# krukah/robopoker

Hardware: AMD Instinct MI355X
Metric: mccfr_infoset_updates_per_sec (higher is better)
Workload: dtype f32; 1 GPU; leduc-holdem external-sampling MCCFR, tables resident in HBM (BASELINE configs[1]); regret=floored, weight=linear, sampling=external, batch_per_gpu=8388608, global_batch=8388608, infosets=120, actions=2, update=composed, parallelism=tree-sharded x1

## Files before the change

include/rp_mi355x.h:

```cpp
#ifndef RP_MI355X_H
#define RP_MI355X_H

#include <stddef.h>
#include <stdint.h>

#ifdef __cplusplus
extern "C" {
#endif

#define RP_API __attribute__((visibility("default")))

typedef enum rp_status {
    RP_OK = 0,
    RP_ERR_INVALID = 1,
    RP_ERR_NO_DEVICE = 2,
    RP_ERR_HIP = 3,
    RP_ERR_UNSUPPORTED = 4,
    RP_ERR_CAPACITY = 5,
    RP_ERR_INTERNAL = 6
} rp_status;

RP_API const char* rp_last_error(void);
RP_API int rp_device_count(void);
RP_API const char* rp_version(void);
// ... 125 lines not shown
RP_API int rp_mccfr_get(rp_mccfr* h, uint32_t info, uint32_t edge, rp_encounter* out);
RP_API int rp_mccfr_set(rp_mccfr* h, uint32_t info, uint32_t edge, const rp_encounter* in);
RP_API int rp_mccfr_export(rp_mccfr* h, rp_encounter* rows, uint64_t cap);
RP_API int rp_mccfr_import(rp_mccfr* h, const rp_encounter* rows, uint64_t n, uint64_t epoch);
typedef enum rp_dist_kind {
    RP_DIST_ITERATED = 0,
    RP_DIST_AVERAGED = 1,
    RP_DIST_SAMPLING = 2
} rp_dist_kind;
RP_API int rp_mccfr_policy(rp_mccfr* h, uint32_t info, rp_dist_kind kind, float* out, uint32_t* n);
RP_API int rp_mccfr_exploitability(rp_mccfr* h, float* out);
RP_API int rp_mccfr_sum_regret(rp_mccfr* h, float* out);
RP_API int rp_mccfr_set_batch(rp_mccfr* h, uint32_t batch_size);
RP_API int rp_mccfr_set_update_mode(rp_mccfr* h, rp_update_mode mode);
RP_API int rp_mccfr_set_stream(rp_mccfr* h, void* hip_stream);

RP_API int rp_mccfr_set_shard(rp_mccfr* h, uint32_t rank, uint32_t world);
RP_API int rp_mccfr_summary_bytes(rp_mccfr* h, size_t* bytes);
RP_API int rp_mccfr_step_local(rp_mccfr* h, void* summary_dev);
RP_API int rp_mccfr_step_apply(rp_mccfr* h, const void* gathered_dev, uint32_t world);
RP_API int rp_mccfr_window_local(rp_mccfr* h, void* window_dev, int first);
RP_API int rp_mccfr_window_apply(rp_mccfr* h, const void* gathered_dev, uint32_t world);

#define RP_COMM_ID_BYTES 128
typedef struct rp_comm rp_comm;
RP_API int rp_comm_unique_id(uint8_t* id );
RP_API int rp_comm_create(const uint8_t* id, int rank, int world, int device, rp_comm** out);
RP_API int rp_comm_adopt(void* nccl_comm, int rank, int world, int device, rp_comm** out);
RP_API int rp_comm_destroy(rp_comm* c);
RP_API int rp_mccfr_step_comm(rp_mccfr* h, rp_comm* c, uint32_t steps, uint32_t window);

RP_API int rp_mccfr_traversal_variant(rp_mccfr* h, int* out);
RP_API int rp_mccfr_traversal_rows_bytes(rp_mccfr* h, size_t* out);
RP_API int rp_game_skeleton(const rp_game_table* game, int* out);

#define RP_SPARSE_BLOCK 64u
typedef struct rp_profile rp_profile;
typedef struct rp_decisions {
    uint32_t n;
    const uint32_t* row;
    const uint8_t* n_actions;
    const uint16_t* expanded;
    const float* regret;
    const float* policy;
    const float* payoff;
} rp_decisions;
RP_API int rp_profile_create(int device, uint64_t n_rows, uint32_t max_actions, rp_regret_kind regret,
                             rp_weight_kind weight, const rp_hyper* hp, const float* default_regret,
                             uint32_t max_batch, rp_profile** out);
RP_API int rp_profile_destroy(rp_profile* h);
RP_API int rp_profile_apply(rp_profile* h, const rp_decisions* batch, rp_update_mode mode);
RP_API int rp_profile_sync(rp_profile* h);
RP_API int rp_profile_epoch(const rp_profile* h, uint64_t* epoch);
RP_API int rp_profile_set_epoch(rp_profile* h, uint64_t epoch);
RP_API int rp_profile_get_rows(rp_profile* h, uint64_t n, const uint32_t* rows, rp_encounter* out);
RP_API int rp_profile_set_rows(rp_profile* h, uint64_t n, const uint32_t* rows, const rp_encounter* in);
RP_API int rp_profile_policy(rp_profile* h, rp_dist_kind kind, uint64_t n, const uint32_t* rows_dev, const uint8_t* n_actions_dev,
                             float* policy_dev);
RP_API int rp_profile_set_stream(rp_profile* h, void* hip_stream);
RP_API int rp_profile_entry_bytes(const rp_profile* h, size_t* bytes);
RP_API int rp_profile_summarize(rp_profile* h, const rp_decisions* batch, void* entries_dev, uint32_t* n_entries);
RP_API int rp_profile_fold(rp_profile* h, const void* entries_dev, uint32_t n_entries);

typedef struct rp_nlhe rp_nlhe;
typedef struct rp_lookup rp_lookup;
RP_API int rp_nlhe_create(int device, uint32_t cap_log2, rp_regret_kind regret, rp_weight_kind weight, const rp_hyper* hp,
// ... 465 lines not shown
```

robopoker_amd/_lib.py:

```python
from __future__ import annotations

import ctypes as C
import os

_HERE = os.path.dirname(os.path.abspath(__file__))
LIB_PATH = os.path.join(_HERE, "librp_mi355x.so")

RP_OK = 0
RP_ERR_INVALID = 1
RP_ERR_NO_DEVICE = 2
RP_ERR_HIP = 3
RP_ERR_UNSUPPORTED = 4
RP_ERR_CAPACITY = 5

RP_TURN_CHANCE = 254
RP_TURN_TERMINAL = 255
RP_NO_INFO = 0xFFFFFFFF

REGRET = {"summed": 0, "linear": 1, "discounted": 2, "floored": 3, "asymmetric": 4}
WEIGHT = {"constant": 0, "linear": 1, "quadratic": 2, "exponential": 3}
SAMPLING = {"external": 0, "prunable": 1, "pluribus": 2}
GAME = {"kuhn": 0, "leduc": 1, "rps": 2, "leduc_wide": 3}
DIST = {"iterated": 0, "averaged": 1, "sampling": 2}
METRIC = {"sinkhorn": 0, "variation": 1}
# ... 248 lines not shown
    "rp_game_table_check": (C.c_int, [C.POINTER(GameTable)]),
    "rp_mccfr_create": (
        C.c_int,
        [C.POINTER(GameTable), C.c_int, C.c_int, C.c_int, C.c_uint32, C.POINTER(Hyper), C.c_uint64, C.c_int,
         C.POINTER(C.c_void_p)],
    ),
    "rp_mccfr_create_mode": (
        C.c_int,
        [C.POINTER(GameTable), C.c_int, C.c_int, C.c_int, C.c_uint32, C.POINTER(Hyper), C.c_uint64, C.c_int, C.c_int,
         C.POINTER(C.c_void_p)],
    ),
    "rp_mccfr_destroy": (C.c_int, [C.c_void_p]),
    "rp_mccfr_step": (C.c_int, [C.c_void_p]),
    "rp_mccfr_solve": (C.c_int, [C.c_void_p, C.c_uint64]),
    "rp_mccfr_spend": (C.c_int, [C.c_void_p, C.c_double, C.POINTER(C.c_uint64), C.POINTER(C.c_double)]),
    "rp_mccfr_step_async": (C.c_int, [C.c_void_p, C.c_uint32]),
    "rp_mccfr_sync": (C.c_int, [C.c_void_p]),
    "rp_mccfr_epoch": (C.c_int, [C.c_void_p, C.POINTER(C.c_uint64)]),
    "rp_mccfr_counters": (C.c_int, [C.c_void_p, C.POINTER(C.c_uint64), C.POINTER(C.c_uint64)]),
    "rp_mccfr_get": (C.c_int, [C.c_void_p, C.c_uint32, C.c_uint32, C.POINTER(Encounter)]),
    "rp_mccfr_set": (C.c_int, [C.c_void_p, C.c_uint32, C.c_uint32, C.POINTER(Encounter)]),
    "rp_mccfr_export": (C.c_int, [C.c_void_p, C.POINTER(Encounter), C.c_uint64]),
    "rp_mccfr_import": (C.c_int, [C.c_void_p, C.POINTER(Encounter), C.c_uint64, C.c_uint64]),
    "rp_mccfr_policy": (C.c_int, [C.c_void_p, C.c_uint32, C.c_int, C.POINTER(C.c_float), C.POINTER(C.c_uint32)]),
    "rp_mccfr_exploitability": (C.c_int, [C.c_void_p, C.POINTER(C.c_float)]),
    "rp_mccfr_sum_regret": (C.c_int, [C.c_void_p, C.POINTER(C.c_float)]),
    "rp_mccfr_set_batch": (C.c_int, [C.c_void_p, C.c_uint32]),
    "rp_mccfr_set_update_mode": (C.c_int, [C.c_void_p, C.c_int]),
    "rp_mccfr_set_rng": (C.c_int, [C.c_void_p, C.c_int, C.POINTER(HashStreams)]),
    "rp_game_hash_streams": (C.c_int, [C.c_void_p, C.POINTER(HashStreams)]),
    "rp_mccfr_set_stream": (C.c_int, [C.c_void_p, C.c_void_p]),
    "rp_mccfr_traversal_variant": (C.c_int, [C.c_void_p, C.POINTER(C.c_int)]),
    "rp_mccfr_traversal_rows_bytes": (C.c_int, [C.c_void_p, C.POINTER(C.c_size_t)]),
    "rp_game_skeleton": (C.c_int, [C.c_void_p, C.POINTER(C.c_int)]),
    "rp_mccfr_set_shard": (C.c_int, [C.c_void_p, C.c_uint32, C.c_uint32]),
    "rp_mccfr_summary_bytes": (C.c_int, [C.c_void_p, C.POINTER(C.c_size_t)]),
    "rp_mccfr_step_local": (C.c_int, [C.c_void_p, C.c_void_p]),
    "rp_mccfr_step_apply": (C.c_int, [C.c_void_p, C.c_void_p, C.c_uint32]),
    "rp_mccfr_window_local": (C.c_int, [C.c_void_p, C.c_void_p, C.c_int]),
    "rp_mccfr_window_apply": (C.c_int, [C.c_void_p, C.c_void_p, C.c_uint32]),
    "rp_comm_unique_id": (C.c_int, [C.c_void_p]),
    "rp_comm_create": (C.c_int, [C.c_void_p, C.c_int, C.c_int, C.c_int, C.POINTER(C.c_void_p)]),
    "rp_comm_adopt": (C.c_int, [C.c_void_p, C.c_int, C.c_int, C.c_int, C.POINTER(C.c_void_p)]),
    "rp_comm_destroy": (C.c_int, [C.c_void_p]),
    "rp_mccfr_step_comm": (C.c_int, [C.c_void_p, C.c_void_p, C.c_uint32, C.c_uint32]),
    "rp_kmeans_step_comm": (C.c_int, [C.c_void_p, C.c_void_p, C.c_void_p, C.c_void_p, C.POINTER(C.c_double)]),
    "rp_mccfr_profile": (C.c_int, [C.c_void_p, C.c_int]),
    "rp_mccfr_kernel_time": (C.c_int, [C.c_void_p, C.c_char_p, C.POINTER(C.c_double), C.POINTER(C.c_uint64)]),
    "rp_profile_create": (C.c_int, [C.c_int, C.c_uint64, C.c_uint32, C.c_int, C.c_int, C.POINTER(Hyper), C.c_void_p, C.c_uint32,
                                    C.POINTER(C.c_void_p)]),
    "rp_profile_destroy": (C.c_int, [C.c_void_p]),
    "rp_profile_apply": (C.c_int, [C.c_void_p, C.POINTER(Decisions), C.c_int]),
    "rp_profile_sync": (C.c_int, [C.c_void_p]),
    "rp_profile_epoch": (C.c_int, [C.c_void_p, C.POINTER(C.c_uint64)]),
    "rp_profile_set_epoch": (C.c_int, [C.c_void_p, C.c_uint64]),
    "rp_profile_get_rows": (C.c_int, [C.c_void_p, C.c_uint64, C.c_void_p, C.c_void_p]),
    "rp_profile_policy": (C.c_int, [C.c_void_p, C.c_int, C.c_uint64, C.c_void_p, C.c_void_p, C.c_void_p]),
    "rp_profile_set_stream": (C.c_int, [C.c_void_p, C.c_void_p]),
    "rp_profile_entry_bytes": (C.c_int, [C.c_void_p, C.POINTER(C.c_size_t)]),
    "rp_profile_summarize": (C.c_int, [C.c_void_p, C.POINTER(Decisions), C.c_void_p, C.POINTER(C.c_uint32)]),
    "rp_profile_fold": (C.c_int, [C.c_void_p, C.c_void_p, C.c_uint32]),
    "rp_profile_profile": (C.c_int, [C.c_void_p, C.c_int]),
    "rp_profile_kernel_time": (C.c_int, [C.c_void_p, C.c_char_p, C.POINTER(C.c_double), C.POINTER(C.c_uint64)]),
    "rp_sinkhorn_hp_default": (None, [C.POINTER(SinkhornHP)]),
    "rp_kmeans_create": (
        C.c_int,
# ... 183 lines not shown
```

robopoker_amd/csrc/mccfr.hip:

```cpp
#include "mccfr_kernels.hpp"
#include "mccfr_traverse.hpp"
#include "mccfr_update.hpp"
#include "traverse_static.hpp"

#include <algorithm>
#include <chrono>
#include <cstdlib>
#include <functional>
#include <string>
#include <type_traits>
#include <vector>

#define HIP_TRY(expr)                                                                                 \
    do {                                                                                              \
        hipError_t _e = (expr);                                                                       \
        if (_e != hipSuccess) return rp::fail(RP_ERR_HIP, "%s failed: %s", #expr, hipGetErrorString(_e)); \
    } while (0)

using namespace rp;

struct KernelClock {
    std::vector<std::pair<hipEvent_t, hipEvent_t>> pending;
    double total_ms = 0.0;
    uint64_t launches = 0;
// ... 22 lines not shown
    void* d_info_actions = nullptr;
    void* d_info_player = nullptr;
    void* d_info_rank = nullptr;
    void* d_scratch = nullptr;
    void* d_dec = nullptr;
    void* d_summary = nullptr;
    void* d_window = nullptr;
    uint32_t window_world = 0;
    void* d_sorted = nullptr;
    void* d_bmaps = nullptr;
    uint32_t maxint = 1;
    void* d_itab = nullptr;
    DevInfoTab itab{};
    DevSorted so{};
    unsigned long long* d_counters = nullptr;
    int R = 0, W = 0, S = 0;
    rp_hyper hp{};
    uint64_t seed = 0;
    rp_rng_kind rng = RP_RNG_COUNTER;
    uint32_t n_chance_infos = 0;
    void* d_info_streams = nullptr;
    void* d_chance_streams = nullptr;
    void* d_ref_mid = nullptr;
    uint64_t ref_mid_epoch = ~0ull;
    uint32_t batch = 1, capacity = 0;
    uint64_t epoch = 0;
    uint32_t rank = 0, world = 1;
    uint32_t maxdec = 1;
    rp_update_mode mode = RP_UPDATE_ORDERED;
    bool use_lds_traverse = false;
    uint64_t tables_version = 1, itab_version = 0;
    static constexpr uint32_t cell_pad = 7;
    bool fuse_maps = true;
    int static_skel = 0;
    bool profiling = false;
    KernelClock clk_traverse, clk_compact, clk_update;
};

namespace {

int set_device(const rp_mccfr* h) {
    HIP_TRY(hipSetDevice(h->device));
    return RP_OK;
}

size_t chain_lds_bytes() { return (size_t)CHAIN_LDS_WORDS * 4; }

size_t summary_bytes_of(const rp_mccfr* h) {
    return (size_t)h->tbl.n_infos * h->tbl.max_actions * sizeof(Cell) + (size_t)h->tbl.n_infos * sizeof(InfoSum);
}

void sampled_tree_bounds(const rp_mccfr* h, uint32_t* maxdec, uint32_t* maxstack, uint32_t* maxint) {
    const rp::TableBounds b = rp::table_bounds(h->tbl, h->tbl.train_root);
    *maxdec = std::max(b.decisions, 1u);
    *maxstack = std::max(b.stack, 1u) + 1;
    *maxint = std::max(b.internal, 1u);
}

size_t chunk_maps_lds_bytes(const rp_mccfr* h);
int alloc_batch_buffers(rp_mccfr* h, uint32_t batch) {
    if (batch <= h->capacity) return RP_OK;
    if (h->d_scratch) HIP_TRY(hipFree(h->d_scratch));
    if (h->d_dec) HIP_TRY(hipFree(h->d_dec));
    h->d_scratch = h->d_dec = nullptr;
    const size_t stride = ((size_t)batch + 255) & ~(size_t)255;
    const uint32_t A = h->tbl.max_actions;
// ... 294 lines not shown

int launch_chain(rp_mccfr* h, const StepParams& p) {
    const size_t lds = chain_lds_bytes();
    const bool sgn = h->R == RP_REGRET_DISCOUNTED || h->R == RP_REGRET_ASYMMETRIC;
    const bool prn = h->S != RP_SAMPLING_EXTERNAL;
    const dim3 grid(h->tbl.n_infos), block(128);
    clock_begin(h, h->clk_update);
    with_bools(sgn, prn, [&](auto sg, auto pr) {
        hipLaunchKernelGGL((k_chain<decltype(sg)::value, decltype(pr)::value>), grid, block, lds, h->stream, h->g, h->t, h->so, p);
    });
    clock_end(h, h->clk_update);
    HIP_TRY(hipGetLastError());
    return RP_OK;
}

uint32_t chunks_of(size_t trees) { return (uint32_t)((trees + RP_COMPOSE_CHUNK - 1) / RP_COMPOSE_CHUNK); }
size_t chunk_maps_lds_bytes(const rp_mccfr* h) {
    const size_t NI = h->tbl.n_infos;
    return NI * SM_WORDS * 4 + 2 * NI * 4 + (size_t)CH_TREES * h->maxdec * 4 + NI * SM_WORDS * 2 +
           2 * (size_t)CH_TREES * h->maxdec * 2;
}

size_t traverse_maps_lds_bytes(const rp_mccfr* h) {
    const size_t NI = h->tbl.n_infos;
    const size_t masks = h->S != RP_SAMPLING_EXTERNAL ? (size_t)h->maxdec * 256 * 4 : 0;
    return (NI * 8 + 2 * NI) * 4 + NI * 8 * 2 + (NI + (NI & 1)) * 2 + 2 * NI * 4 + (size_t)3 * (h->maxdec * 256 + h->cell_pad) * 4 + masks;
}
static_assert(CH_THREADS <= 256u, "k_traverse_maps_static packs (infoset, rank of the infoset) into the 16 bits of an `order` entry");
bool traverse_maps_fused(const rp_mccfr* h) {
    return h->static_skel && !h->dc.slotmap && h->tbl.n_infos <= CH_THREADS && h->g.rank_max <= 64u &&
           traverse_maps_lds_bytes(h) <= 64 * 1024 && h->fuse_maps;
}

int launch_summarize(rp_mccfr* h, const StepParams& p, void* blob_dev, bool fused = false, bool apply = false) {
    unsigned char* blob = reinterpret_cast<unsigned char*>(blob_dev);
    Cell* cells = reinterpret_cast<Cell*>(blob);
    InfoSum* sums = reinterpret_cast<InfoSum*>(blob + (size_t)h->tbl.n_infos * h->tbl.max_actions * sizeof(Cell));
    const uint32_t A = h->tbl.max_actions;
    const uint32_t nblk_max = chunks_of(h->dc.stride), nblk = chunks_of(h->batch);
    Map* bmaps = reinterpret_cast<Map*>(h->d_bmaps);
    const bool pruned = h->S != RP_SAMPLING_EXTERNAL;
    if (fused) {
        clock_begin(h, h->clk_traverse);
        launch_prepare(h, p);
        const size_t lds = traverse_maps_lds_bytes(h);
        with_static_traversal(h->static_skel, p.walker, pruned, p.ref_info != nullptr, [&](auto gt, auto wk, auto pr, auto rf) {
            hipLaunchKernelGGL((k_traverse_maps_static<decltype(gt), decltype(wk)::value, decltype(pr)::value, decltype(rf)::value>), dim3(nblk),
                               dim3(256), lds, h->stream, h->g, h->itab, p, bmaps, h->maxdec, h->cell_pad);
        });
        clock_end(h, h->clk_traverse);
    }
    clock_begin(h, h->clk_update);
    if (fused) {
    } else if (!h->dc.slotmap) {
        const size_t lds = chunk_maps_lds_bytes(h);
        with_bools(pruned, h->tbl.n_infos <= CH_THREADS, [&](auto pr, auto one) {
            hipLaunchKernelGGL((k_chunk_maps<decltype(pr)::value, decltype(one)::value ? 1u : CM_PASSES>), dim3(nblk), dim3(CH_THREADS), lds,
                               h->stream, h->g, h->dc, p, bmaps);
        });
    } else {
        with_bool(pruned, [&](auto pr) {
            hipLaunchKernelGGL((k_block_maps<decltype(pr)::value>), dim3(nblk, h->tbl.n_infos), dim3(128), 0, h->stream, h->g, h->so, p, bmaps);
        });
    }
    {
        const uint32_t W2 = 2 * A, nr = h->g.rank_count[p.walker];
        const uint32_t ngrp_max = (nblk_max + RP_FOLD_GROUP - 1) / RP_FOLD_GROUP, ngrp = (nblk + RP_FOLD_GROUP - 1) / RP_FOLD_GROUP;
        FoldScratch fs;
        fs.gmaps = bmaps + bmap_index(nblk_max, 0, 0, h->g.rank_max, W2);
        fs.done = reinterpret_cast<uint32_t*>(bmaps + bmap_index(nblk_max + ngrp_max, 0, 0, h->g.rank_max, W2));
        const dim3 grid(std::max(ngrp, 1u), cb2_tiles(nr, W2));
        if (apply) {
            hipLaunchKernelGGL((k_combine2<true>), grid, dim3(CB2_THREADS), 0, h->stream, h->g, h->t, h->itab, p, bmaps, nr, fs, cells, sums);
            h->tables_version += 1;
            if (h->itab_version + 1 == h->tables_version) h->itab_version = h->tables_version;
        } else {
            hipLaunchKernelGGL((k_combine2<false>), grid, dim3(CB2_THREADS), 0, h->stream, h->g, h->t, h->itab, p, bmaps, nr, fs, cells, sums);
        }
    }
    clock_end(h, h->clk_update);
    HIP_TRY(hipGetLastError());
    return RP_OK;
}

int launch_batch_summary(rp_mccfr* h, const StepParams& p, void* blob_dev, bool apply = false) {
    if (traverse_maps_fused(h)) return launch_summarize(h, p, blob_dev, true, apply);
    int rc = launch_traverse(h, p);
    if (rc) return rc;
    if (h->dc.slotmap && (rc = launch_sort(h, p))) return rc;
    return launch_summarize(h, p, blob_dev, false, apply);
}

int enqueue_step(rp_mccfr* h) {
    const StepParams p = make_params(h);
    int rc;
    if (h->mode == RP_UPDATE_ORDERED) {
        if ((rc = launch_traverse(h, p))) return rc;
        if ((rc = launch_sort(h, p))) return rc;
        if ((rc = launch_chain(h, p))) return rc;
        h->tables_version += 1;
    } else {
        if ((rc = launch_batch_summary(h, p, h->d_summary, true))) return rc;
    }
    h->epoch += 1;
    return RP_OK;
}

int read_counters(rp_mccfr* h, unsigned long long c[3]) {
    std::vector<unsigned long long> all((size_t)METRIC_STRIPES * METRIC_STRIDE);
    HIP_TRY(hipMemcpyAsync(all.data(), h->d_counters, all.size() * 8, hipMemcpyDeviceToHost, h->stream));
// ... 154 lines not shown
    CREATE_TRY(hipMemset(h->t.weight, 0, cells * 4));
    CREATE_TRY(hipMemset(h->t.payoff, 0, cells * 4));
    CREATE_TRY(hipMemset(h->t.visits, 0, cells * 4));
    CREATE_TRY(hipMalloc(&h->d_counters, (size_t)METRIC_STRIPES * METRIC_STRIDE * sizeof(unsigned long long)));
    CREATE_TRY(hipMemset(h->d_counters, 0, (size_t)METRIC_STRIPES * METRIC_STRIDE * sizeof(unsigned long long)));
    CREATE_TRY(hipMalloc(&h->d_summary, summary_bytes_of(h)));
    CREATE_TRY(hipMalloc(&h->d_itab, (5 * cells + 2 * (size_t)game->n_infos + 4 + 8 * (size_t)game->n_infos + 8) * 4));
    {
        float* f = reinterpret_cast<float*>(h->d_itab);
        h->itab.sigma = f;
        h->itab.q = f + cells;
        h->itab.cum = f + 2 * cells;
        h->itab.total = f + 3 * cells;
        h->itab.keep = reinterpret_cast<uint32_t*>(f + 3 * cells + game->n_infos);
        const size_t used = 3 * cells + 2 * (size_t)game->n_infos;
        h->itab.sq = reinterpret_cast<float2*>(f + ((used + 3) & ~(size_t)3));
        const size_t used2 = ((used + 3) & ~(size_t)3) + 2 * cells;
        h->itab.row2 = game->max_actions == 2 ? f + ((used2 + 7) & ~(size_t)7) : nullptr;
    }
    uint32_t maxstack = 1;
    sampled_tree_bounds(h, &h->maxdec, &maxstack, &h->maxint);
    h->sc.maxn = game->max_tree_nodes;
    h->sc.maxs = maxstack;
    if (h->maxdec > 254) {
        rp_mccfr_destroy(h);
        return rp::fail(RP_ERR_CAPACITY, "rp_mccfr_create: more than 254 walker infosets per tree");
    }
    if (chain_lds_bytes() > 64 * 1024) {
        rp_mccfr_destroy(h);
        return rp::fail(RP_ERR_CAPACITY, "rp_mccfr_create: chain tiles need %zu B of LDS", chain_lds_bytes());
    }
    h->use_lds_traverse = traverse_fits_lds(h) && getenv("RP_MCCFR_HBM_SCRATCH") == nullptr;
    h->fuse_maps = getenv("RP_TRAV_UNFUSED") == nullptr;
    if (h->use_lds_traverse && getenv("RP_TRAV_GENERIC") == nullptr) {
        for (int k = 1; k <= 2 && !h->static_skel; ++k)
            with_skeleton(k, [&](auto gt) {
                if (skel_matches<decltype(gt)>(game, h->children)) h->static_skel = k;
            });
    }
    h->g.rows = nullptr;
    if (h->static_skel && getenv("RP_TRAV_NO_FLAT") == nullptr) {
        std::vector<uint32_t> rows;
        bool ok = false;
        with_skeleton(h->static_skel, [&](auto gt) { ok = build_rows<decltype(gt)>(game, h->children, rec_of, rows, h->g.row_base, h->g.row_fan); });
        if (ok) {
            CREATE_TRY(hipMalloc(&h->d_rows, rows.size() * 4));
            CREATE_TRY(hipMemcpy(h->d_rows, rows.data(), rows.size() * 4, hipMemcpyHostToDevice));
            h->g.rows = reinterpret_cast<const uint4*>(h->d_rows);
            h->rows_bytes = rows.size() * 4;
        }
    }
    rc = alloc_batch_buffers(h, batch_size);
    if (rc) {
        rp_mccfr_destroy(h);
        return rc;
    }
#undef CREATE_TRY
    (void)hipDeviceSynchronize();
    *out = h;
    return RP_OK;
}

int rp_mccfr_destroy(rp_mccfr* h) {
    if (!h) return RP_OK;
    (void)hipSetDevice(h->device);
    if (h->stream) (void)hipStreamSynchronize(h->stream);
// ... 418 lines not shown

int rp_mccfr_profile(rp_mccfr* h, int enable) {
    if (!h) return rp::fail(RP_ERR_INVALID, "rp_mccfr_profile: NULL handle");
    (void)hipSetDevice(h->device);
    (void)hipStreamSynchronize(h->stream);
    clock_drain_all(h);
    h->profiling = enable != 0;
    h->clk_traverse.total_ms = h->clk_compact.total_ms = h->clk_update.total_ms = 0.0;
    h->clk_traverse.launches = h->clk_compact.launches = h->clk_update.launches = 0;
    return RP_OK;
}

int rp_game_skeleton(const rp_game_table* game, int* out) {
    if (!game || !out) return rp::fail(RP_ERR_INVALID, "rp_game_skeleton: NULL argument");
    int rc = rp_game_table_check(game);
    if (rc) return rc;
    const std::vector<uint32_t> children(game->children, game->children + game->n_children);
    *out = skel_matches<KuhnSkel>(game, children) ? 1 : (skel_matches<LeducSkel>(game, children) ? 2 : 0);
    return RP_OK;
}

int rp_mccfr_traversal_rows_bytes(rp_mccfr* h, size_t* out) {
    if (!h || !out) return rp::fail(RP_ERR_INVALID, "rp_mccfr_traversal_rows_bytes: NULL argument");
    *out = h->rows_bytes;
    return RP_OK;
}

int rp_mccfr_traversal_variant(rp_mccfr* h, int* out) {
    if (!h || !out) return rp::fail(RP_ERR_INVALID, "rp_mccfr_traversal_variant: NULL argument");
    *out = h->static_skel ? 2 : (h->use_lds_traverse ? 1 : 0);
    return RP_OK;
}

int rp_mccfr_kernel_time(rp_mccfr* h, const char* name, double* total_ms, uint64_t* launches) {
    if (!h || !name) return rp::fail(RP_ERR_INVALID, "rp_mccfr_kernel_time: NULL argument");
    (void)hipSetDevice(h->device);
    (void)hipStreamSynchronize(h->stream);
    clock_drain_all(h);
    const KernelClock* c = nullptr;
    if (std::string(name) == "traverse") c = &h->clk_traverse;
    else if (std::string(name) == "compact") c = &h->clk_compact;
    else if (std::string(name) == "update") c = &h->clk_update;
    else return rp::fail(RP_ERR_INVALID, "rp_mccfr_kernel_time: unknown kernel '%s'", name);
    if (total_ms) *total_ms = c->total_ms;
    if (launches) *launches = c->launches;
    return RP_OK;
}

namespace {
struct XNode {
    uint32_t state;
    int32_t parent, edge;
    int32_t kids[RP_MAX_ACTIONS];
};
struct XCtx {
    const rp_mccfr* h;
    const float* weight;
    std::vector<XNode> nodes;
    float wt(uint32_t info, uint32_t a) const { return rp_maxf(weight[(size_t)info * h->tbl.max_actions + a], RP_EPSILON); }
    float averaged(uint32_t info, uint32_t a) const {
        float sum = 0.0f;
        for (uint32_t k = 0; k < h->info_actions[info]; ++k) sum += wt(info, k);
        return wt(info, a) / sum;
    }
    float value(int32_t n, uint32_t hero, const int32_t* br) const {
        const XNode& nd = nodes[n];
// ... 83 lines not shown
```

robopoker_amd/csrc/mccfr_update.hpp:

```cpp
#ifndef RP_MCCFR_UPDATE_HPP
#define RP_MCCFR_UPDATE_HPP

#include "mccfr_kernels.hpp"
#include "mccfr_traverse.hpp"

namespace rp {

#define CH_THREADS 256u
#define SLOT_THREADS (CH_TREES / 4u)

__device__ __forceinline__ uint32_t chunk_slots(const DevDecisions& dc, uint32_t info, uint32_t t0, uint32_t batch) {
    uint32_t slots = 0;
    if (t0 + 4 <= batch) {
        slots = *reinterpret_cast<const uint32_t*>(&dc.slotmap[(size_t)info * dc.stride + t0]);
    } else {
        for (uint32_t k = 0; k < 4; ++k)
            if (t0 + k < batch) slots |= (uint32_t)dc.slotmap[(size_t)info * dc.stride + t0 + k] << (8 * k);
    }
    return slots;
}
__device__ __forceinline__ uint32_t nonzero_bytes(uint32_t v) {
    return ((v & 0xffu) != 0) + ((v & 0xff00u) != 0) + ((v & 0xff0000u) != 0) + ((v & 0xff000000u) != 0);
}
__device__ __forceinline__ uint32_t block_exscan(uint32_t v, uint32_t* wave_tot, uint32_t* total) {
// ... 556 lines not shown
                for (uint32_t e = 0; e < n; ++e)
                    map_touch_unless(mp, PRUNED && isreg && !((lmask[base + e] >> a) & 1u), cp.d, vals[base + e], cp.fl);
            bmaps[out] = mp;
        }
    }
}

#if defined(__HIP_DEVICE_COMPILE__) && !defined(__gfx950__) && !defined(__gfx942__)
#error "k_combine2's cross-workgroup hand-over relies on gfx942/gfx950 store counting and sc1 semantics: use an acq_rel arrival counter on other targets"
#endif
__device__ __forceinline__ void st_agent(uint32_t* q, uint32_t v) { __hip_atomic_store(q, v, __ATOMIC_RELAXED, __HIP_MEMORY_SCOPE_AGENT); }
__device__ __forceinline__ void st_map(Map* m, const Map& v) {
    uint32_t* w = reinterpret_cast<uint32_t*>(m);
    st_agent(w, rp_f2u(v.a));
    st_agent(w + 1, rp_f2u(v.b));
    st_agent(w + 2, rp_f2u(v.m));
    st_agent(w + 3, v.n);
}
#ifndef CB2_DEPTH
#define CB2_DEPTH 8u
#endif
#ifndef CB2_DEPTH2
#define CB2_DEPTH2 8u
#endif
#define CB2_THREADS 256u
static_assert(2u * RP_MAX_ACTIONS + 1u <= CB2_THREADS, "a tile of k_combine2 holds at least one whole infoset");
__host__ __device__ inline uint32_t cb2_tile_infos(uint32_t W2) { return CB2_THREADS / (W2 + 1u); }
__host__ __device__ inline uint32_t cb2_tiles(uint32_t nr, uint32_t W2) { return nr ? (nr + cb2_tile_infos(W2) - 1u) / cb2_tile_infos(W2) : 1u; }
struct FoldScratch {
    Map* gmaps;
    uint32_t* done;
};
template <uint32_t D, class Load>
__device__ __forceinline__ Map fold_slots(uint32_t n, bool sum, Load load) {
    Map m = map_identity();
    uint4 va[D], vb[D];
    auto issue = [&](uint4* v, uint32_t k0) __attribute__((always_inline)) {
#pragma unroll
        for (uint32_t q = 0; q < D; ++q) v[q] = load(min(k0 + q, n - 1u));
    };
    auto fold = [&](const uint4* v, uint32_t k0) __attribute__((always_inline)) {
#pragma unroll
        for (uint32_t q = 0; q < D; ++q) {
            const Map s{rp_u2f(v[q].x), rp_u2f(v[q].y), rp_u2f(v[q].z), v[q].w};
            const Map c = map_compose_select(m, s);
            const bool on = k0 + q < n;
            m.a = on ? c.a : m.a;
            m.b = on ? (sum ? m.b + s.b : c.b) : m.b;
            m.m = on ? c.m : m.m;
            m.n = on ? m.n + s.n : m.n;
        }
    };
    uint32_t k0 = 0;
    issue(va, 0u);
    for (; k0 + 2u * D < n; k0 += 2u * D) {
        issue(vb, k0 + D);
        __builtin_amdgcn_sched_barrier(0);
        fold(va, k0);
        __builtin_amdgcn_sched_barrier(0);
        issue(va, k0 + 2u * D);
        __builtin_amdgcn_sched_barrier(0);
        fold(vb, k0 + D);
        __builtin_amdgcn_sched_barrier(0);
    }
    if (k0 + D < n) {
        issue(vb, k0 + D);
        __builtin_amdgcn_sched_barrier(0);
        fold(va, k0);
        fold(vb, k0 + D);
    } else {
        fold(va, k0);
    }
    return m;
}
template <bool APPLY>
__global__ __launch_bounds__(CB2_THREADS) void k_combine2(DevGame g, DevTables t, DevInfoTab it, StepParams p, const Map* bmaps, uint32_t nr,
                                                          FoldScratch fs, Cell* cells, InfoSum* sums) {
    __shared__ uint32_t role;
    __shared__ float sh_ps[CB2_THREADS / 3u];
    __shared__ uint32_t sh_len[CB2_THREADS / 3u];
    const uint32_t grp = blockIdx.x, tile = blockIdx.y, tid = threadIdx.x;
    const uint32_t A = g.A, W2 = 2 * A, SL = W2 + 1u;
    if (!APPLY && grp == 0 && tile == 0) {
        const Map ident = map_identity();
        for (uint32_t e = tid; e < g.n_infos * SL; e += CB2_THREADS) {
            const uint32_t info = e / SL, slot = e - info * SL;
            if (g.info_player[info] == p.walker) continue;
            if (slot == W2) {
                sums[info] = InfoSum{0u, 0.0f};
            } else {
                Cell& cl = cells[(size_t)info * A + slot % A];
                if (slot < A) cell_set_regret(cl, ident);
                else cell_set_weight(cl, ident);
            }
        }
    }
    const uint32_t nb = (p.batch + RP_COMPOSE_CHUNK - 1) / RP_COMPOSE_CHUNK;
    const uint32_t ngrp = (nb + RP_FOLD_GROUP - 1) / RP_FOLD_GROUP;
    if (grp >= ngrp) return;
    const uint32_t ntiles = cb2_tiles(nr, W2);
    const uint32_t r_lo = (uint32_t)((uint64_t)tile * nr / ntiles), r_hi = (uint32_t)((uint64_t)(tile + 1u) * nr / ntiles);
    const uint32_t li = tid / SL, slot = tid - li * SL, rank = r_lo + li;
    const bool active = rank < r_hi, sum = slot == W2;
    const size_t row = (size_t)g.rank_max * SL;
    if (active) {
        const uint32_t b_lo = grp * RP_FOLD_GROUP, n = min(nb, b_lo + RP_FOLD_GROUP) - b_lo;
        const uint4* src = reinterpret_cast<const uint4*>(bmaps) + bmap_index(b_lo, rank, slot, g.rank_max, W2);
        const Map m = fold_slots<CB2_DEPTH>(n, sum, [&](uint32_t k) { return src[(size_t)k * row]; });
        st_map(&fs.gmaps[bmap_index(grp, rank, slot, g.rank_max, W2)], m);
    }
    asm volatile("s_waitcnt vmcnt(0)" ::: "memory");
    __syncthreads();
    if (tid == 0) role = atomicAdd(&fs.done[tile], 1u) == ngrp - 1u ? 1u : 0u;
    __syncthreads();
    if (!role) return;
    if (tid == 0) fs.done[tile] = 0;
    Map tot = map_identity();
    uint32_t info = 0;
    if (active) {
        const uint64_t* gm = reinterpret_cast<const uint64_t*>(fs.gmaps + bmap_index(0u, rank, slot, g.rank_max, W2));
        tot = fold_slots<CB2_DEPTH2>(ngrp, sum, [&](uint32_t k) {
            const uint64_t* w = gm + (size_t)k * row * 2u;
            const uint64_t lo = __hip_atomic_load(w, __ATOMIC_RELAXED, __HIP_MEMORY_SCOPE_AGENT);
            const uint64_t hi = __hip_atomic_load(w + 1, __ATOMIC_RELAXED, __HIP_MEMORY_SCOPE_AGENT);
            return make_uint4((uint32_t)lo, (uint32_t)(lo >> 32), (uint32_t)hi, (uint32_t)(hi >> 32));
        });
        info = g.rank_info[(size_t)p.walker * g.rank_max + rank];
    }
    if (!APPLY) {
        if (active) {
            if (sum) {
                sums[info] = InfoSum{tot.n, tot.b};
            } else {
                Cell& cl = cells[(size_t)info * A + slot % A];
                if (slot < A) cell_set_regret(cl, tot);
                else cell_set_weight(cl, tot);
            }
        }
        return;
    }
    if (active && sum) {
        sh_ps[li] = tot.b;
        sh_len[li] = tot.n;
    }
    __syncthreads();
    if (active && !sum && slot % A < g.info_actions[info]) {
        const uint32_t cell = info * A + slot % A;
        if (slot < A) {
            t.regret[cell] = map_apply(tot, t.regret[cell]);
            float ev = t.payoff[cell];
            uint32_t visits = t.visits[cell];
            fold_payoff(ev, visits, sh_ps[li], sh_len[li]);
            t.payoff[cell] = ev;
            t.visits[cell] = visits;
        } else {
            t.weight[cell] = map_apply(tot, t.weight[cell]);
        }
    }
    __syncthreads();
    if (active && slot == 0) prepare_one(g, t, p, it, info);
}

__global__ void k_fold(DevGame g, DevTables t, const unsigned char* blob, size_t blob_stride, uint32_t world) {
    const uint32_t cell = blockIdx.x * blockDim.x + threadIdx.x;
    const uint32_t ncell = g.n_infos * g.A;
    if (cell >= ncell) return;
    const uint32_t info = cell / g.A, a = cell % g.A;
    if (a >= g.info_actions[info]) return;
    float r = t.regret[cell], w = t.weight[cell], ev = t.payoff[cell];
    uint32_t visits = t.visits[cell];
    for (uint32_t rk = 0; rk < world; ++rk) {
        const unsigned char* b = blob + (size_t)rk * blob_stride;
        const Cell c = reinterpret_cast<const Cell*>(b)[cell];
        const InfoSum s = reinterpret_cast<const InfoSum*>(b + (size_t)ncell * sizeof(Cell))[info];
        if (c.rn) r = map_eval(cell_regret(c), r);
        if (c.wn) w = map_eval(cell_weight(c), w);
        fold_payoff(ev, visits, s.psum, s.count);
    }
    t.regret[cell] = r;
    t.weight[cell] = w;
    t.payoff[cell] = ev;
    t.visits[cell] = visits;
}

__global__ void k_accumulate(DevGame g, unsigned char* acc, const unsigned char* step, uint32_t first) {
    const uint32_t cell = blockIdx.x * blockDim.x + threadIdx.x;
    const uint32_t ncell = g.n_infos * g.A;
    if (cell >= ncell) return;
    const Cell s = reinterpret_cast<const Cell*>(step)[cell];
    Cell* ac = reinterpret_cast<Cell*>(acc) + cell;
    if (first) {
        *ac = s;
    } else {
// ... 18 lines not shown
```

robopoker_amd/mccfr.py:

```python
from __future__ import annotations

import ctypes as C

import numpy as np

from . import _lib
from .games import Game

ENC_DTYPE = np.dtype([("weight", "<f4"), ("regret", "<f4"), ("payoff", "<f4"), ("visits", "<u4")])


def default_hyper() -> _lib.Hyper:
    hp = _lib.Hyper()
    _lib.load().rp_hyper_default(C.byref(hp))
    return hp


class Solver:

    def __init__(self, game: Game, regret="floored", weight="linear", sampling="external", batch=1, seed=0,
                 hyper=None, device=0, mode=None):
        self._lib = _lib.load()
        self.game = game
        self.hp = hyper if hyper is not None else default_hyper()
# ... 117 lines not shown
        _lib.check(self._lib.rp_mccfr_set_stream(self._h, C.c_void_p(hip_stream_ptr)))

    def set_shard(self, rank: int, world: int):
        _lib.check(self._lib.rp_mccfr_set_shard(self._h, rank, world))

    def summary_bytes(self) -> int:
        n = C.c_size_t()
        _lib.check(self._lib.rp_mccfr_summary_bytes(self._h, C.byref(n)))
        return n.value

    def step_local(self, summary_dev_ptr: int):
        _lib.check(self._lib.rp_mccfr_step_local(self._h, C.c_void_p(summary_dev_ptr)))

    def step_apply(self, gathered_dev_ptr: int, world: int):
        _lib.check(self._lib.rp_mccfr_step_apply(self._h, C.c_void_p(gathered_dev_ptr), world))

    def window_local(self, window_dev_ptr: int, first: bool):
        _lib.check(self._lib.rp_mccfr_window_local(self._h, C.c_void_p(window_dev_ptr), 1 if first else 0))

    def window_apply(self, gathered_dev_ptr: int, world: int):
        _lib.check(self._lib.rp_mccfr_window_apply(self._h, C.c_void_p(gathered_dev_ptr), world))

    def step_comm(self, comm, steps: int, window: int = 1):
        _lib.check(self._lib.rp_mccfr_step_comm(self._h, comm.handle, steps, window))

    def profile(self, enable=True):
        _lib.check(self._lib.rp_mccfr_profile(self._h, 1 if enable else 0))

    def kernel_variant(self) -> str:
        v = C.c_int()
        _lib.check(self._lib.rp_mccfr_traversal_variant(self._h, C.byref(v)))
        return ("hbm", "lds", "static")[v.value]

    def traversal_rows_bytes(self) -> int:
        n = C.c_size_t()
        _lib.check(self._lib.rp_mccfr_traversal_rows_bytes(self._h, C.byref(n)))
        return n.value

    def kernel_time(self, name: str):
        ms, n = C.c_double(), C.c_uint64()
        _lib.check(self._lib.rp_mccfr_kernel_time(self._h, name.encode(), C.byref(ms), C.byref(n)))
        return ms.value, n.value
```

Baseline: 81.99 billion infoset-updates/s.

## Split the map fold into a group-fold stage and a per-rank slab fold kernel

For large batches, the fused combine kernel, which uses an atomic counter to elect a last block that folds all group maps, is replaced by two launches. Stage one writes per-group maps with plain stores. A new k_fold_groups kernel then launches one block per rank, stages group maps through an LDS slab and folds them before applying updates. This aims to remove the serialized last-block tail and the atomic handoff, at the cost of an extra kernel launch and a round trip through global memory.

```diff
diff --git a/include/rp_mi355x.h b/include/rp_mi355x.h
--- a/include/rp_mi355x.h
+++ b/include/rp_mi355x.h
@@ -181,6 +181,7 @@
 
 RP_API int rp_mccfr_traversal_variant(rp_mccfr* h, int* out);
 RP_API int rp_mccfr_traversal_rows_bytes(rp_mccfr* h, size_t* out);
+RP_API int rp_mccfr_fold_variant(rp_mccfr* h, int* out);
 RP_API int rp_game_skeleton(const rp_game_table* game, int* out);
 
 #define RP_SPARSE_BLOCK 64u
diff --git a/robopoker_amd/_lib.py b/robopoker_amd/_lib.py
--- a/robopoker_amd/_lib.py
+++ b/robopoker_amd/_lib.py
@@ -304,6 +304,7 @@
     "rp_mccfr_set_stream": (C.c_int, [C.c_void_p, C.c_void_p]),
     "rp_mccfr_traversal_variant": (C.c_int, [C.c_void_p, C.POINTER(C.c_int)]),
     "rp_mccfr_traversal_rows_bytes": (C.c_int, [C.c_void_p, C.POINTER(C.c_size_t)]),
+    "rp_mccfr_fold_variant": (C.c_int, [C.c_void_p, C.POINTER(C.c_int)]),
     "rp_game_skeleton": (C.c_int, [C.c_void_p, C.POINTER(C.c_int)]),
     "rp_mccfr_set_shard": (C.c_int, [C.c_void_p, C.c_uint32, C.c_uint32]),
     "rp_mccfr_summary_bytes": (C.c_int, [C.c_void_p, C.POINTER(C.c_size_t)]),
diff --git a/robopoker_amd/csrc/mccfr.hip b/robopoker_amd/csrc/mccfr.hip
--- a/robopoker_amd/csrc/mccfr.hip
+++ b/robopoker_amd/csrc/mccfr.hip
@@ -78,6 +78,7 @@
     uint64_t tables_version = 1, itab_version = 0;
     static constexpr uint32_t cell_pad = 7;
     bool fuse_maps = true;
+    uint32_t fold_split_groups = 0;
     int static_skel = 0;
     bool profiling = false;
     KernelClock clk_traverse, clk_compact, clk_update;
@@ -438,6 +439,12 @@
            traverse_maps_lds_bytes(h) <= 64 * 1024 && h->fuse_maps;
 }
 
+constexpr uint32_t FOLD_SPLIT_GROUPS = 128;
+bool fold_split(const rp_mccfr* h, uint32_t batch) {
+    const uint32_t ngrp = (chunks_of(batch) + RP_FOLD_GROUP - 1) / RP_FOLD_GROUP;
+    return ngrp >= h->fold_split_groups;
+}
+
 int launch_summarize(rp_mccfr* h, const StepParams& p, void* blob_dev, bool fused = false, bool apply = false) {
     unsigned char* blob = reinterpret_cast<unsigned char*>(blob_dev);
     Cell* cells = reinterpret_cast<Cell*>(blob);
@@ -475,13 +482,17 @@
         FoldScratch fs;
         fs.gmaps = bmaps + bmap_index(nblk_max, 0, 0, h->g.rank_max, W2);
         fs.done = reinterpret_cast<uint32_t*>(bmaps + bmap_index(nblk_max + ngrp_max, 0, 0, h->g.rank_max, W2));
-        const dim3 grid(std::max(ngrp, 1u), cb2_tiles(nr, W2));
+        const dim3 grid(std::max(ngrp, 1u), cb2_tiles(nr, W2)), fold_grid(std::max(nr, 1u));
+        const bool split = fold_split(h, h->batch);
+        if (split) hipLaunchKernelGGL((k_combine2<false, false>), grid, dim3(CB2_THREADS), 0, h->stream, h->g, h->t, h->itab, p, bmaps, nr, fs, cells, sums);
         if (apply) {
-            hipLaunchKernelGGL((k_combine2<true>), grid, dim3(CB2_THREADS), 0, h->stream, h->g, h->t, h->itab, p, bmaps, nr, fs, cells, sums);
+            if (split) hipLaunchKernelGGL((k_fold_groups<true>), fold_grid, dim3(CB2_THREADS), 0, h->stream, h->g, h->t, h->itab, p, fs.gmaps, nr, cells, sums);
+            else hipLaunchKernelGGL((k_combine2<true>), grid, dim3(CB2_THREADS), 0, h->stream, h->g, h->t, h->itab, p, bmaps, nr, fs, cells, sums);
             h->tables_version += 1;
             if (h->itab_version + 1 == h->tables_version) h->itab_version = h->tables_version;
         } else {
-            hipLaunchKernelGGL((k_combine2<false>), grid, dim3(CB2_THREADS), 0, h->stream, h->g, h->t, h->itab, p, bmaps, nr, fs, cells, sums);
+            if (split) hipLaunchKernelGGL((k_fold_groups<false>), fold_grid, dim3(CB2_THREADS), 0, h->stream, h->g, h->t, h->itab, p, fs.gmaps, nr, cells, sums);
+            else hipLaunchKernelGGL((k_combine2<false>), grid, dim3(CB2_THREADS), 0, h->stream, h->g, h->t, h->itab, p, bmaps, nr, fs, cells, sums);
         }
     }
     clock_end(h, h->clk_update);
@@ -702,6 +713,8 @@
     }
     h->use_lds_traverse = traverse_fits_lds(h) && getenv("RP_MCCFR_HBM_SCRATCH") == nullptr;
     h->fuse_maps = getenv("RP_TRAV_UNFUSED") == nullptr;
+    const char* fold_env = getenv("RP_FOLD_SPLIT");
+    h->fold_split_groups = !fold_env ? FOLD_SPLIT_GROUPS : (atoi(fold_env) ? 1u : UINT32_MAX);
     if (h->use_lds_traverse && getenv("RP_TRAV_GENERIC") == nullptr) {
         for (int k = 1; k <= 2 && !h->static_skel; ++k)
             with_skeleton(k, [&](auto gt) {
@@ -1186,6 +1199,12 @@
     return RP_OK;
 }
 
+int rp_mccfr_fold_variant(rp_mccfr* h, int* out) {
+    if (!h || !out) return rp::fail(RP_ERR_INVALID, "rp_mccfr_fold_variant: NULL argument");
+    *out = fold_split(h, h->batch) ? 1 : 0;
+    return RP_OK;
+}
+
 int rp_mccfr_kernel_time(rp_mccfr* h, const char* name, double* total_ms, uint64_t* launches) {
     if (!h || !name) return rp::fail(RP_ERR_INVALID, "rp_mccfr_kernel_time: NULL argument");
     (void)hipSetDevice(h->device);
diff --git a/robopoker_amd/csrc/mccfr_update.hpp b/robopoker_amd/csrc/mccfr_update.hpp
--- a/robopoker_amd/csrc/mccfr_update.hpp
+++ b/robopoker_amd/csrc/mccfr_update.hpp
@@ -612,8 +612,7 @@
     uint32_t* done;
 };
 template <uint32_t D, class Load>
-__device__ __forceinline__ Map fold_slots(uint32_t n, bool sum, Load load) {
-    Map m = map_identity();
+__device__ __forceinline__ Map fold_slots(Map m, uint32_t n, bool sum, Load load) {
     uint4 va[D], vb[D];
     auto issue = [&](uint4* v, uint32_t k0) __attribute__((always_inline)) {
 #pragma unroll
@@ -653,28 +652,69 @@
     }
     return m;
 }
+__device__ __forceinline__ void blob_idle_entries(const DevGame& g, const StepParams& p, Cell* cells, InfoSum* sums) {
+    const uint32_t A = g.A, W2 = 2 * A, SL = W2 + 1u;
+    const Map ident = map_identity();
+    for (uint32_t e = threadIdx.x; e < g.n_infos * SL; e += CB2_THREADS) {
+        const uint32_t info = e / SL, slot = e - info * SL;
+        if (g.info_player[info] == p.walker) continue;
+        if (slot == W2) {
+            sums[info] = InfoSum{0u, 0.0f};
+        } else {
+            Cell& cl = cells[(size_t)info * A + slot % A];
+            if (slot < A) cell_set_regret(cl, ident);
+            else cell_set_weight(cl, ident);
+        }
+    }
+}
 template <bool APPLY>
+__device__ __forceinline__ void fold_finish(const DevGame& g, const DevTables& t, const DevInfoTab& it, const StepParams& p, bool active, uint32_t li,
+                                            uint32_t slot, uint32_t info, const Map& tot, Cell* cells, InfoSum* sums, float* sh_ps, uint32_t* sh_len) {
+    const uint32_t A = g.A, W2 = 2 * A;
+    const bool sum = slot == W2;
+    if (!APPLY) {
+        if (active) {
+            if (sum) {
+                sums[info] = InfoSum{tot.n, tot.b};
+            } else {
+                Cell& cl = cells[(size_t)info * A + slot % A];
+                if (slot < A) cell_set_regret(cl, tot);
+                else cell_set_weight(cl, tot);
+            }
+        }
+        return;
+    }
+    if (active && sum) {
+        sh_ps[li] = tot.b;
+        sh_len[li] = tot.n;
+    }
+    __syncthreads();
+    if (active && !sum && slot % A < g.info_actions[info]) {
+        const uint32_t cell = info * A + slot % A;
+        if (slot < A) {
+            t.regret[cell] = map_apply(tot, t.regret[cell]);
+            float ev = t.payoff[cell];
+            uint32_t visits = t.visits[cell];
+            fold_payoff(ev, visits, sh_ps[li], sh_len[li]);
+            t.payoff[cell] = ev;
+            t.visits[cell] = visits;
+        } else {
+            t.weight[cell] = map_apply(tot, t.weight[cell]);
+        }
+    }
+    __syncthreads();
+    if (active && slot == 0) prepare_one(g, t, p, it, info);
+}
+template <bool APPLY, bool TAIL = true>
 __global__ __launch_bounds__(CB2_THREADS) void k_combine2(DevGame g, DevTables t, DevInfoTab it, StepParams p, const Map* bmaps, uint32_t nr,
                                                           FoldScratch fs, Cell* cells, InfoSum* sums) {
+    static_assert(TAIL || !APPLY, "stage 1 alone applies nothing");
     __shared__ uint32_t role;
     __shared__ float sh_ps[CB2_THREADS / 3u];
     __shared__ uint32_t sh_len[CB2_THREADS / 3u];
     const uint32_t grp = blockIdx.x, tile = blockIdx.y, tid = threadIdx.x;
     const uint32_t A = g.A, W2 = 2 * A, SL = W2 + 1u;
-    if (!APPLY && grp == 0 && tile == 0) {
-        const Map ident = map_identity();
-        for (uint32_t e = tid; e < g.n_infos * SL; e += CB2_THREADS) {
-            const uint32_t info = e / SL, slot = e - info * SL;
-            if (g.info_player[info] == p.walker) continue;
-            if (slot == W2) {
-                sums[info] = InfoSum{0u, 0.0f};
-            } else {
-                Cell& cl = cells[(size_t)info * A + slot % A];
-                if (slot < A) cell_set_regret(cl, ident);
-                else cell_set_weight(cl, ident);
-            }
-        }
-    }
+    if (TAIL && !APPLY && grp == 0 && tile == 0) blob_idle_entries(g, p, cells, sums);
     const uint32_t nb = (p.batch + RP_COMPOSE_CHUNK - 1) / RP_COMPOSE_CHUNK;
     const uint32_t ngrp = (nb + RP_FOLD_GROUP - 1) / RP_FOLD_GROUP;
     if (grp >= ngrp) return;
@@ -686,9 +726,11 @@
     if (active) {
         const uint32_t b_lo = grp * RP_FOLD_GROUP, n = min(nb, b_lo + RP_FOLD_GROUP) - b_lo;
         const uint4* src = reinterpret_cast<const uint4*>(bmaps) + bmap_index(b_lo, rank, slot, g.rank_max, W2);
-        const Map m = fold_slots<CB2_DEPTH>(n, sum, [&](uint32_t k) { return src[(size_t)k * row]; });
-        st_map(&fs.gmaps[bmap_index(grp, rank, slot, g.rank_max, W2)], m);
-    }
+        const Map m = fold_slots<CB2_DEPTH>(map_identity(), n, sum, [&](uint32_t k) { return src[(size_t)k * row]; });
+        if (TAIL) st_map(&fs.gmaps[bmap_index(grp, rank, slot, g.rank_max, W2)], m);
+        else fs.gmaps[bmap_index(grp, rank, slot, g.rank_max, W2)] = m;
+    }
+    if (!TAIL) return;
     asm volatile("s_waitcnt vmcnt(0)" ::: "memory");
     __syncthreads();
     if (tid == 0) role = atomicAdd(&fs.done[tile], 1u) == ngrp - 1u ? 1u : 0u;
@@ -699,7 +741,7 @@
     uint32_t info = 0;
     if (active) {
         const uint64_t* gm = reinterpret_cast<const uint64_t*>(fs.gmaps + bmap_index(0u, rank, slot, g.rank_max, W2));
-        tot = fold_slots<CB2_DEPTH2>(ngrp, sum, [&](uint32_t k) {
+        tot = fold_slots<CB2_DEPTH2>(tot, ngrp, sum, [&](uint32_t k) {
             const uint64_t* w = gm + (size_t)k * row * 2u;
             const uint64_t lo = __hip_atomic_load(w, __ATOMIC_RELAXED, __HIP_MEMORY_SCOPE_AGENT);
             const uint64_t hi = __hip_atomic_load(w + 1, __ATOMIC_RELAXED, __HIP_MEMORY_SCOPE_AGENT);
@@ -707,38 +749,53 @@
         });
         info = g.rank_info[(size_t)p.walker * g.rank_max + rank];
     }
-    if (!APPLY) {
-        if (active) {
-            if (sum) {
-                sums[info] = InfoSum{tot.n, tot.b};
-            } else {
-                Cell& cl = cells[(size_t)info * A + slot % A];
-                if (slot < A) cell_set_regret(cl, tot);
-                else cell_set_weight(cl, tot);
-            }
-        }
-        return;
-    }
-    if (active && sum) {
-        sh_ps[li] = tot.b;
-        sh_len[li] = tot.n;
-    }
-    __syncthreads();
-    if (active && !sum && slot % A < g.info_actions[info]) {
-        const uint32_t cell = info * A + slot % A;
-        if (slot < A) {
-            t.regret[cell] = map_apply(tot, t.regret[cell]);
-            float ev = t.payoff[cell];
-            uint32_t visits = t.visits[cell];
-            fold_payoff(ev, visits, sh_ps[li], sh_len[li]);
-            t.payoff[cell] = ev;
-            t.visits[cell] = visits;
-        } else {
-            t.weight[cell] = map_apply(tot, t.weight[cell]);
-        }
-    }
-    __syncthreads();
-    if (active && slot == 0) prepare_one(g, t, p, it, info);
+    fold_finish<APPLY>(g, t, it, p, active, li, slot, info, tot, cells, sums, sh_ps, sh_len);
+}
+
+#define FG_LOADS 10u
+#define FG_SLOTS (FG_LOADS * CB2_THREADS)
+#define FG_DEPTH 8u
+static_assert(2u * RP_MAX_ACTIONS + 1u <= FG_SLOTS, "a slab of k_fold_groups holds at least one group");
+__host__ __device__ inline uint32_t fg_slab_groups(uint32_t W2) { return FG_SLOTS / (W2 + 1u); }
+template <bool APPLY>
+__global__ __launch_bounds__(CB2_THREADS) void k_fold_groups(DevGame g, DevTables t, DevInfoTab it, StepParams p, const Map* gmaps, uint32_t nr,
+                                                             Cell* cells, InfoSum* sums) {
+    typedef uint32_t __attribute__((ext_vector_type(4))) Word4;
+    __shared__ __attribute__((aligned(16))) Word4 slab[FG_SLOTS];
+    __shared__ float sh_ps[1];
+    __shared__ uint32_t sh_len[1];
+    const uint32_t rank = blockIdx.x, tid = threadIdx.x;
+    const uint32_t A = g.A, W2 = 2 * A, SL = W2 + 1u;
+    if (!APPLY && rank == 0) blob_idle_entries(g, p, cells, sums);
+    if (rank >= nr) return;
+    const uint32_t nb = (p.batch + RP_COMPOSE_CHUNK - 1) / RP_COMPOSE_CHUNK;
+    const uint32_t ngrp = (nb + RP_FOLD_GROUP - 1) / RP_FOLD_GROUP, per = fg_slab_groups(W2);
+    const size_t row = (size_t)g.rank_max * SL;
+    const Word4* src = reinterpret_cast<const Word4*>(gmaps) + bmap_index(0u, rank, 0u, g.rank_max, W2);
+    const bool active = tid < SL;
+    Map tot = map_identity();
+    for (uint32_t g0 = 0; g0 < ngrp; g0 += per) {
+        const uint32_t n = min(per, ngrp - g0), nel = n * SL;
+        Word4 v[FG_LOADS];
+#pragma unroll
+        for (uint32_t q = 0; q < FG_LOADS; ++q) {
+            const uint32_t e = min(tid + q * CB2_THREADS, nel - 1u), k = e / SL;
+            v[q] = src[(size_t)(g0 + k) * row + (e - k * SL)];
+        }
+        if (g0) __syncthreads();
+#pragma unroll
+        for (uint32_t q = 0; q < FG_LOADS; ++q) {
+            const uint32_t e = tid + q * CB2_THREADS;
+            if (e < nel) slab[e] = v[q];
+        }
+        __syncthreads();
+        if (active) tot = fold_slots<FG_DEPTH>(tot, n, tid == W2, [&](uint32_t k) {
+            const Word4 w = slab[k * SL + tid];
+            return make_uint4(w.x, w.y, w.z, w.w);
+        });
+    }
+    const uint32_t info = g.rank_info[(size_t)p.walker * g.rank_max + rank];
+    fold_finish<APPLY>(g, t, it, p, active, 0u, tid, info, tot, cells, sums, sh_ps, sh_len);
 }
 
 __global__ void k_fold(DevGame g, DevTables t, const unsigned char* blob, size_t blob_stride, uint32_t world) {
diff --git a/robopoker_amd/mccfr.py b/robopoker_amd/mccfr.py
--- a/robopoker_amd/mccfr.py
+++ b/robopoker_amd/mccfr.py
@@ -173,6 +173,11 @@
         _lib.check(self._lib.rp_mccfr_traversal_variant(self._h, C.byref(v)))
         return ("hbm", "lds", "static")[v.value]
 
+    def fold_variant(self) -> str:
+        v = C.c_int()
+        _lib.check(self._lib.rp_mccfr_fold_variant(self._h, C.byref(v)))
+        return ("fused", "split")[v.value]
+
     def traversal_rows_bytes(self) -> int:
         n = C.c_size_t()
         _lib.check(self._lib.rp_mccfr_traversal_rows_bytes(self._h, C.byref(n)))
```

New measurement: 85.97 billion infoset-updates/s, median of 6. +4.9%, better.
